# antao97/SegGroup

Measured on AMD Instinct MI355X. Metric: pseudo-label scenes/sec (150k pts, 1.5k segs), higher is better.
Workload: dtype f32 (fp32 accumulate; operands split into 2 x fp16 pieces on v_mfma_f32_32x32x16_f16; kNN / FPS scores in exact fp32 order); 1 GPU; 64 distinct synthetic scenes per GPU per step, 150000 pts / 1500 segs each (BASELINE.json configs[2]; configs[1] = the same scene shape, single scene); mode=ins_infer, scenes_in_flight=112, engine=14 groups x 8 scenes per batched launch, weights=tests/golden/weights_g2.npz, parallelism=scene-parallel x1

## Files before the change

### include/seggroup_hip.h

```cpp
#ifndef SEGGROUP_HIP_H
#define SEGGROUP_HIP_H

#include <stddef.h>
#include <stdint.h>

#ifdef __cplusplus
extern "C" {
#endif

#define SG_OK          0
#define SG_EINVAL     -1
#define SG_EHIP       -2
#define SG_ENOMEM     -3
#define SG_ESTALL     -4
#define SG_EUNSUP     -5
#define SG_EINTERNAL  -6

#define SG_MODE_INS_INFER 0
#define SG_MODE_SEM_INFER 1

#define SG_NUM_LABEL_VECTORS 14
#define SG_RANGE_WORDS 256
#define SG_MAX_POINTS (1 << 20)

const char* sg_last_error(void);
int  sg_version(void);
int  sg_device_count(void);
int  sg_selftest_wave_ops(int* h_mismatches, void* stream);
int  sg_selftest_list_insert(int* h_mismatches, void* stream);

size_t sg_contract_ws_bytes(int S);
int sg_contract_point_edges(const int64_t* d_adj, int E, const int32_t* d_seg_of_point, int N, int S,
                            int32_t* d_out_adj, int out_capacity, int32_t* d_out_count,
                            void* d_ws, size_t ws_bytes, void* stream);

int sg_gather_members(const int32_t* d_seg_points, const int32_t* d_seg_off, int S,
                      const int32_t* d_order, const int32_t* d_dst, const int32_t* d_cl,
                      int32_t* d_members, int32_t* d_pos_of_point, int32_t* d_cluster_of_pos,
                      int32_t* d_slot_of_pos, void* stream);

size_t sg_fps_ws_bytes(int N);
int sg_fps_sample(const float* d_data, int N, int ch_in, const int32_t* d_members, const int32_t* d_cl_off, int C,
                  int P, int ch_out, int transform, float* d_samples, int32_t* d_sel,
                  void* d_ws, size_t ws_bytes, void* stream);

size_t sg_mlp1_ws_bytes(int C);
int sg_mlp1_forward(const float* d_samples, int C, const float* d_w, const float* d_gamma, const float* d_beta,
                    float* d_feat, int feat_stride, void* d_ws, size_t ws_bytes, void* stream);

int sg_edge_distance(const float* d_feat, int feat_stride, int D, const int32_t* d_adj, int E,
                     float* d_dist, void* stream);

int sg_group_max_rows(const float* d_rows, int row_stride, int D, const int32_t* d_goff, const int32_t* d_gidx,
                      int G, float* d_out, int out_stride, void* stream);

int sg_segment_max(const float* d_rows, int N, int D, const int32_t* d_cluster_of_pos,
                   float* d_out, int out_stride, int C, void* stream);

size_t sg_center_ws_bytes(int T, int C);
int sg_center_clusters(const float* d_data, int N, const int32_t* d_members, const int32_t* d_cl_off, int C,
                       const int32_t* d_tile_cl, const int32_t* d_tile_lo, const int32_t* d_tile_hi, int T,
                       const int32_t* d_cl_tile_off, float* d_x9m, float* d_xyzw,
                       void* d_ws, size_t ws_bytes, void* stream);

int sg_cluster_knn(const float* d_xyzw, int N, const int32_t* d_cl_off,
                   const int32_t* d_tile_cl, const int32_t* d_tile_lo, const int32_t* d_tile_hi, int T,
                   int k, int pos0, int32_t* d_knn, void* stream);

int sg_segment_boxes(const float* d_data, const int32_t* d_seg_points, const int32_t* d_seg_off, int S,
                     float* d_box, void* stream);
int sg_cluster_knn_pruned(const float* d_xyzw, int N, const int32_t* d_cl_off,
                          const int32_t* d_tile_cl, const int32_t* d_tile_lo, const int32_t* d_tile_hi, int T,
                          const int32_t* d_cl_seg_off, const int32_t* d_order, const int32_t* d_dst,
                          const int32_t* d_seg_off, const float* d_segbox, const int32_t* d_slot_of_pos,
                          int k, int pos0, int32_t* d_knn, void* stream);

size_t sg_segment_sort_ws_bytes(int N);
int sg_segment_sort_boxes(const float* d_data, int N, const int32_t* d_seg_points, const int32_t* d_seg_off,
                          const int32_t* d_seg_of_point, int S, const int32_t* d_seg_chunk_off, int max_seg, float* d_segbox,
                          int32_t* d_sperm, float* d_chunk_box, double* d_seg_sums, void* d_ws, size_t ws_bytes, void* stream);
int sg_layer_layout(const float* d_data, int N, const int32_t* d_seg_points, const int32_t* d_seg_off, const int32_t* d_sperm, int S,
                    const int32_t* d_order, const int32_t* d_dst, const int32_t* d_cl, const float* d_cl_mean, int32_t* d_members,
                    int32_t* d_pos_of_point, int32_t* d_cluster_of_pos, int32_t* d_slot_of_pos, float* d_x9m, float* d_sxyzw,
                    int32_t* d_smpos, float* d_point_rec, int32_t* d_seed_id, unsigned int* d_range_bits, void* stream);
int sg_knn_operands(const float* d_data, const int32_t* d_seg_points, const int32_t* d_seg_off, const int32_t* d_sperm, int S,
                    const int32_t* d_order, const int32_t* d_dst, float* d_sxyzw, int32_t* d_smpos, void* stream);
int sg_cluster_knn_sorted(const float* d_sxyzw, const int32_t* d_smpos, int N, const int32_t* d_cl_off,
                          const int32_t* d_tile_cl, const int32_t* d_tile_lo, const int32_t* d_tile_hi, int T,
                          const int32_t* d_cl_seg_off, const int32_t* d_order, const int32_t* d_dst,
                          const int32_t* d_seg_off, const int32_t* d_seg_chunk_off, const float* d_segbox,
                          const float* d_chunk_box, const int32_t* d_slot_of_pos, int k, int pos0, int32_t* d_knn, void* stream);
int sg_knn_seed_points(const int32_t* d_knn, const int32_t* d_members, int N, int k, int32_t* d_seed, void* stream);
int sg_cluster_knn_seeded(const float* d_sxyzw, const int32_t* d_smpos, int N, const int32_t* d_cl_off,
                          const int32_t* d_tile_cl, const int32_t* d_tile_lo, const int32_t* d_tile_hi, int T,
                          const int32_t* d_cl_seg_off, const int32_t* d_order, const int32_t* d_dst,
                          const int32_t* d_seg_off, const int32_t* d_seg_chunk_off, const float* d_segbox,
                          const float* d_chunk_box, const int32_t* d_slot_of_pos, const int32_t* d_seed,
                          const int32_t* d_seg_prevcl, const int32_t* d_members, const float* d_point_rec,
                          int k, int pos0, int32_t* d_knn, void* stream);

int sg_knn_chunk_table(const int32_t* d_order, const int32_t* d_dst, const int32_t* d_seg_off, const int32_t* d_seg_chunk_off,
                       const float* d_chunk_box, int S, const int32_t* d_slot_chunk0, float* d_cc, void* stream);
int sg_cluster_knn_2pass(const float* d_sxyzw, const int32_t* d_smpos, int N, const int32_t* d_cl_off,
                         const int32_t* d_tile_cl, const int32_t* d_tile_lo, const int32_t* d_tile_hi,
                         const int32_t* d_tile_chunk0, int T, const int32_t* d_cl_chunk_off, const float* d_cc,
                         int k, int pos0, int32_t* d_knn, void* stream);
int sg_cluster_knn_sorted_w(const float* d_sxyzw, const int32_t* d_smpos, int N, const int32_t* d_cl_off,
                            const int32_t* d_tile_cl, const int32_t* d_tile_lo, const int32_t* d_tile_hi, int T,
                            const int32_t* d_cl_seg_off, const int32_t* d_order, const int32_t* d_dst,
                            const int32_t* d_seg_off, const int32_t* d_seg_chunk_off, const float* d_segbox,
                            const float* d_chunk_box, const int32_t* d_slot_of_pos, int k, int pos0, int waves_per_tile,
                            int32_t* d_knn, void* stream);

size_t sg_edgeconv_ws_bytes(int N);
int sg_edgeconv_forward(const float* d_x9m, const int32_t* d_knn, int N, int k, int layers,
                        const float* d_w1, const float* d_g1, const float* d_b1,
                        const float* d_w2, const float* d_g2, const float* d_b2,
                        float* d_out, void* d_ws, size_t ws_bytes, void* stream);
int sg_edgeconv_forward_r(const float* d_x9m, const int32_t* d_knn, int N, int k, int layers, const float* d_w1, const float* d_g1,
                          const float* d_b1, const float* d_w2, const float* d_g2, const float* d_b2, float* d_out, void* d_ws,
                          size_t ws_bytes, unsigned int* d_range_bits, void* stream);
#define SG_EDGECONV_COMPILER_LOOP 1u
int sg_edgeconv_forward_x(const float* d_x9m, const int32_t* d_knn, int N, int k, int layers, const float* d_w1, const float* d_g1,
                          const float* d_b1, const float* d_w2, const float* d_g2, const float* d_b2, float* d_out, void* d_ws,
                          size_t ws_bytes, unsigned int* d_range_bits, unsigned int flags, void* stream);
int sg_edge_range(const float* d_x9m, int N, unsigned int* d_range_bits, void* stream);

size_t sg_gcn_ws_bytes(int S, int D, int E);
int sg_gcn_forward(const float* d_x, int S, int D, const int32_t* d_adj, int E,
                   const int32_t* d_rowptr, const int32_t* d_col, const int32_t* d_eid,
// ... 527 lines not shown
```

### seggroup_amd/csrc/kernels_knn_sorted.hip

```cpp
#include <cstdlib>


#include "engine_ctx.h"
#include "knn_device.h"
#include "sg_common.h"
#include "wave_ops.h"

namespace {

using namespace sgknn;

#ifdef SG_KNN_PROFILE
constexpr bool kKnnProfile = true;
#else
constexpr bool kKnnProfile = false;
#endif

constexpr int kChunkPts = 32;
constexpr int kQuadS = 4;

__device__ inline unsigned int spread10(unsigned int v);
__device__ inline unsigned int morton30(const float* __restrict__ r, const float* __restrict__ b) {
    const float e[3] = {b[3] - b[0], b[4] - b[1], b[5] - b[2]};
    const float emax = fmaxf(fmaxf(e[0], e[1]), e[2]);
    unsigned int q[3];
#pragma unroll
    for (int k = 0; k < 3; ++k) {
        const float ext = e[k] >= 0.25f * emax ? e[k] : emax;
        const float t = ext > 0.f ? (r[k] - b[k]) / ext : 0.f;
        q[k] = (unsigned int)fminf(fmaxf(t * 1023.f, 0.f), 1023.f);
    }
    return spread10(q[0]) | (spread10(q[1]) << 1) | (spread10(q[2]) << 2);
}

__device__ inline unsigned int spread10(unsigned int v) {
    v &= 0x3ffu;
    v = (v | (v << 16)) & 0x030000ffu;
    v = (v | (v << 8)) & 0x0300f00fu;
    v = (v | (v << 4)) & 0x030c30c3u;
    v = (v | (v << 2)) & 0x09249249u;
    return v;
}

constexpr int kSortCap = sg::kSegMidMax;
__device__ __forceinline__ void segment_sort_boxes_body(const float* __restrict__ data, const int32_t* __restrict__ seg_points,
                                                        const int32_t* __restrict__ seg_off, const int32_t* __restrict__ seg_chunk_off,
                                                        float* __restrict__ segbox, int32_t* __restrict__ sperm,
                                                        float* __restrict__ chunk_box, double* __restrict__ seg_sums, int s) {
    __shared__ unsigned long long key[kSortCap];
    __shared__ float red[4][8];
    __shared__ double dred[4][3];
    __shared__ float bx[8];
    const int tid = threadIdx.x, lane = tid & 63, wave = tid >> 6;
    const int lo = seg_off[s], n = seg_off[s + 1] - lo;
    if (n > kSortCap) return;
    float mn[3] = {INFINITY, INFINITY, INFINITY}, mx[3] = {-INFINITY, -INFINITY, -INFINITY}, xx = 0.f;
    double sm[3] = {0.0, 0.0, 0.0};
    for (int i = tid; i < n; i += 256) {
        const float* r = data + (size_t)seg_points[lo + i] * 6;
#pragma unroll
        for (int k = 0; k < 3; ++k) { mn[k] = fminf(mn[k], r[k]); mx[k] = fmaxf(mx[k], r[k]); sm[k] += (double)r[k]; }
        xx = fmaxf(xx, (r[0] * r[0] + r[1] * r[1]) + r[2] * r[2]);
    }
#pragma unroll
    for (int k = 0; k < 3; ++k) { mn[k] = sgw::wave_min(mn[k]); mx[k] = sgw::wave_max(mx[k]); }
    xx = sgw::wave_max(xx);
    if (seg_sums) {
#pragma unroll
        for (int k = 0; k < 3; ++k) sm[k] = sgw::wave_sum(sm[k]);
        if (lane == 0) { dred[wave][0] = sm[0]; dred[wave][1] = sm[1]; dred[wave][2] = sm[2]; }
    }
    if (lane == 0) { red[wave][0] = mn[0]; red[wave][1] = mn[1]; red[wave][2] = mn[2]; red[wave][3] = mx[0]; red[wave][4] = mx[1]; red[wave][5] = mx[2]; red[wave][6] = xx; }
    __syncthreads();
    if (tid < 7) {
        float v = red[0][tid];
        for (int w = 1; w < 4; ++w) v = tid < 3 ? fminf(v, red[w][tid]) : fmaxf(v, red[w][tid]);
        bx[tid] = v;
        segbox[(size_t)s * 8 + tid] = v;
    }
    if (tid == 7) segbox[(size_t)s * 8 + 7] = 0.f;
    if (seg_sums && tid >= 8 && tid < 11) seg_sums[(size_t)s * 3 + (tid - 8)] = ((dred[0][tid - 8] + dred[1][tid - 8]) + dred[2][tid - 8]) + dred[3][tid - 8];
    __syncthreads();
    int m2 = 64;
    while (m2 < n) m2 <<= 1;
    for (int i = tid; i < m2; i += 256) {
        unsigned long long kk = ~0ull;
        if (i < n) {
            const float* r = data + (size_t)seg_points[lo + i] * 6;
            const unsigned int m = morton30(r, bx);
            kk = ((unsigned long long)m << 32) | (unsigned int)i;
        }
        key[i] = kk;
    }
    __syncthreads();
    for (int k = 2; k <= m2; k <<= 1)
        for (int j = k >> 1; j > 0; j >>= 1) {
            for (int t = tid; t < (m2 >> 1); t += 256) {
                const int i = ((t & ~(j - 1)) << 1) | (t & (j - 1)), p = i | j;
                const unsigned long long a = key[i], b = key[p];
                const bool up = (i & k) == 0;
                if ((a > b) == up) { key[i] = b; key[p] = a; }
            }
            __syncthreads();
        }
    for (int r = tid; r < n; r += 256) sperm[lo + r] = lo + (int)(key[r] & 0xffffffffull);
    const int c0 = seg_chunk_off[s], half = lane >> 5, l = lane & 31;
    for (int j = 2 * wave + half; j * kChunkPts < n; j += 8) {
        const int t = j * kChunkPts + l;
        float cmn[3] = {INFINITY, INFINITY, INFINITY}, cmx[3] = {-INFINITY, -INFINITY, -INFINITY}, cxx = 0.f;
        if (t < n) {
            const float* r = data + (size_t)seg_points[lo + (int)(key[t] & 0xffffffffull)] * 6;
#pragma unroll
            for (int k = 0; k < 3; ++k) { cmn[k] = r[k]; cmx[k] = r[k]; }
            cxx = (r[0] * r[0] + r[1] * r[1]) + r[2] * r[2];
        }
#pragma unroll
        for (int k = 0; k < 3; ++k) { cmn[k] = sgw::half_min(cmn[k], lane); cmx[k] = sgw::half_max(cmx[k], lane); }
        cxx = sgw::half_max(cxx, lane);
        if (l == 0) {
            float* b = chunk_box + (size_t)(c0 + j) * 8;
            b[0] = cmn[0]; b[1] = cmn[1]; b[2] = cmn[2]; b[3] = cmx[0]; b[4] = cmx[1]; b[5] = cmx[2]; b[6] = cxx; b[7] = 0.f;
        }
    }
}
__global__ __launch_bounds__(256) void k_segment_sort_boxes(const float* __restrict__ data, const int32_t* __restrict__ seg_points,
                                                            const int32_t* __restrict__ seg_off, const int32_t* __restrict__ seg_chunk_off,
                                                            float* __restrict__ segbox, int32_t* __restrict__ sperm,
                                                            float* __restrict__ chunk_box, double* __restrict__ seg_sums) {
    segment_sort_boxes_body(data, seg_points, seg_off, seg_chunk_off, segbox, sperm, chunk_box, seg_sums, blockIdx.x);
}
__global__ __launch_bounds__(256) void k_segment_sort_boxes_b(const sg::SlotCtx* __restrict__ cx) {
    const sg::SlotCtx& c = cx[blockIdx.y];
    if ((int)blockIdx.x >= c.S) return;
    segment_sort_boxes_body(c.data, c.seg_points, c.seg_off, c.seg_chunk_off, c.segbox, c.sperm, c.chunk_box, c.seg_sums, blockIdx.x);
}

constexpr int kBigBlock = 1024, kBins = 4096, kWin = 1024;
constexpr int kBigPieces = 16, kPieceBlock = 256;
struct BigScratch {
    float box[kBigPieces][8];
    double sums[kBigPieces][4];
    int hist[kBins];
    int cursor[kBins];
    int first[kBins];
};
static_assert(kBins % kBigPieces == 0 && kBins / kBigPieces == kPieceBlock, "every piece zeroes its own slice of the histogram: one entry per thread");
__host__ __device__ inline size_t bigseg_scratch_slots(int N) { return (size_t)N / (kSortCap + 1) + 1; }
__device__ __forceinline__ BigScratch& bigseg_scratch(unsigned long long* keysA, int N, int lo) {
    return reinterpret_cast<BigScratch*>(keysA + 2 * (size_t)N)[lo / (kSortCap + 1)];
}
__device__ __forceinline__ void piece_range(int n, int piece, int& i0, int& i1) {
    const int L = (n + kBigPieces - 1) / kBigPieces;
    i0 = min(n, piece * L); i1 = min(n, i0 + L);
}

__device__ __forceinline__ void bigseg_box_body(const float* __restrict__ data, const int32_t* __restrict__ seg_points, const int32_t* __restrict__ seg_off,
                                                unsigned long long* __restrict__ keysA, int N, int s, int piece) {
    const int lo = seg_off[s], n = seg_off[s + 1] - lo;
    if (n <= kSortCap) return;
    BigScratch& sc = bigseg_scratch(keysA, N, lo);
    __shared__ float red[kPieceBlock / 64][8];
    __shared__ double dred[kPieceBlock / 64][3];
    const int tid = threadIdx.x, lane = tid & 63, wave = tid >> 6;
    constexpr int kW = kPieceBlock / 64;
    int i0, i1;
    piece_range(n, piece, i0, i1);
    float mn[3] = {INFINITY, INFINITY, INFINITY}, mx[3] = {-INFINITY, -INFINITY, -INFINITY}, xx = 0.f;
    double sm[3] = {0.0, 0.0, 0.0};
#pragma unroll 4
    for (int i = i0 + tid; i < i1; i += kPieceBlock) {
        const float* r = data + (size_t)seg_points[lo + i] * 6;
#pragma unroll
        for (int k = 0; k < 3; ++k) { mn[k] = fminf(mn[k], r[k]); mx[k] = fmaxf(mx[k], r[k]); sm[k] += (double)r[k]; }
        xx = fmaxf(xx, (r[0] * r[0] + r[1] * r[1]) + r[2] * r[2]);
    }
#pragma unroll
    for (int o = 32; o > 0; o >>= 1) {
#pragma unroll
        for (int k = 0; k < 3; ++k) { mn[k] = fminf(mn[k], __shfl_xor(mn[k], o)); mx[k] = fmaxf(mx[k], __shfl_xor(mx[k], o)); sm[k] += __shfl_xor(sm[k], o); }
        xx = fmaxf(xx, __shfl_xor(xx, o));
    }
    if (lane == 0) {
        red[wave][0] = mn[0]; red[wave][1] = mn[1]; red[wave][2] = mn[2]; red[wave][3] = mx[0]; red[wave][4] = mx[1]; red[wave][5] = mx[2]; red[wave][6] = xx;
        dred[wave][0] = sm[0]; dred[wave][1] = sm[1]; dred[wave][2] = sm[2];
    }
    sc.hist[piece * kPieceBlock + tid] = 0;
    sc.cursor[piece * kPieceBlock + tid] = 0;
// ... 929 lines not shown
    for (int j = 0; j < K; ++j) kv[j] = 0ull;
    {
        const unsigned long long floor_key = make_key(floor_score == 0.f ? -0.f : floor_score, 0x7fffffff) & 0xffffffff00000000ull;
        unsigned long long thr = active ? floor_key - 1ull : ~0ull;
        float wk = active ? floor_score : INFINITY;
#pragma unroll
        for (int o = 32; o > 0; o >>= 1) wk = fminf(wk, __shfl_xor(wk, o));
        int cnt = 0;
        auto drain = [&]() {
            int mxc = cnt;
#pragma unroll
            for (int o = 32; o > 0; o >>= 1) mxc = max(mxc, __shfl_xor(mxc, o));
            for (int u = 0; u < mxc; ++u) key_insert<K>(kv, u < cnt ? buf[u][lane] : 0ull);
            cnt = 0;
            if (active && kv[K - 1] > thr) thr = kv[K - 1];
        };
        walk([&]() { return wk; },
             [&](const float* bx) { return !__any(make_key(box_score_bound(me, bx), 0) > thr); },
             [&](float sc, int idx) {
                 const unsigned long long key = make_key(sc, idx);
                 if (key > thr) {
                     buf[cnt][lane] = key;
                     ++cnt;
                 }
             },
             [&]() { return __any(cnt > kBuf2 - kQuadS - 1); }, drain);
    }
    if (active) {
        int32_t* o = knn + (size_t)myrow * K;
#pragma unroll
        for (int j = 0; j < K; ++j) o[j] = clo + key_index(kv[j]);
    }
    if ((dbg & 16) && lane == 0) {
        const unsigned long long t2 = __builtin_readcyclecounter();
        atomicAdd(&g_knn5_stats[0], 1ull);
        atomicAdd(&g_knn5_stats[1], t1 - t0);
        atomicAdd(&g_knn5_stats[3], t2 - t1);
    }
}

}

int sg::knn_variant_for(int T, int override) {
    if (override == 0 || override == 1 || override == 2 || override == 4 || override == 8) return override;
    return T >= 2048 ? 8 : T >= 1024 ? 2 : 4;
}

namespace sg {

bool sort_boxes_fits_lds(int max_seg) { return max_seg <= kSortCap; }

int b_sort_boxes(const SlotCtx* d_ctx, const BatchDims& bd, hipStream_t st, int which) {
    if (bd.nslots == 0 || bd.max_S == 0) return SG_OK;
    if (which & 1) k_segment_sort_boxes_b<<<dim3(bd.max_S, bd.nslots), 256, 0, st>>>(d_ctx);
    if ((which & 2) && bd.max_big > 0) {
        const int wins = sg::cdiv(bd.max_N, kWin);
        k_bigseg_box_b<<<dim3(bd.max_big * kBigPieces, bd.nslots), kPieceBlock, 0, st>>>(d_ctx);
        k_bigseg_keys_b<<<dim3(bd.max_big * kBigPieces, bd.nslots), kPieceBlock, 0, st>>>(d_ctx);
        k_bigseg_scatter_b<<<dim3(bd.max_big * kBigPieces, bd.nslots), kPieceBlock, 0, st>>>(d_ctx);
        k_bigseg_runs_b<<<dim3(wins, bd.nslots), kBigBlock, 0, st>>>(d_ctx);
        k_bigseg_boxes_b<<<dim3(wins, bd.nslots), 512, 0, st>>>(d_ctx);
    }
    SG_LAUNCH_CHECK();
    return SG_OK;
}

int b_layer_layout(const SlotCtx* d_ctx, const BatchDims& bd, hipStream_t st) {
    if (bd.nslots == 0 || bd.max_S == 0) return SG_OK;
    k_layer_layout_b<<<dim3(bd.max_S, bd.nslots), 256, 0, st>>>(d_ctx);
    if (bd.max_lay_big > 0) k_layer_layout_big_b<<<dim3(bd.max_lay_big, bd.nslots), 256, 0, st>>>(d_ctx);
    SG_LAUNCH_CHECK();
    return SG_OK;
}

int b_cluster_knn(const SlotCtx* d_ctx, const BatchDims& bd, int waves_per_tile, bool seeded, hipStream_t st, bool write_seed, bool* wrote_seed) {
    if (wrote_seed) *wrote_seed = false;
    if (bd.nslots == 0 || bd.max_T == 0) return SG_OK;
    if (bd.max_N > sgknn::kListMaxPoints) return sg::fail(SG_EUNSUP, "in-cluster kNN: %d points in a scene, the list keys carry 20 index bits (N <= %d)", bd.max_N, sgknn::kListMaxPoints);
    const dim3 grid(bd.nslots, bd.max_T);
    if (seeded) k_cluster_knn_sorted_b<20, 1, true><<<grid, 64, 0, st>>>(d_ctx, 0);
    else if (waves_per_tile == 1) {
        k_cluster_knn_sorted_b<20, 1, false><<<grid, 64, 0, st>>>(d_ctx, write_seed ? 1 : 0);
        if (wrote_seed) *wrote_seed = write_seed;
    } else if (waves_per_tile == 2) k_cluster_knn_sorted_b<20, 2, false><<<grid, 128, 0, st>>>(d_ctx, 0);
    else k_cluster_knn_sorted_b<20, 4, false><<<grid, 256, 0, st>>>(d_ctx, 0);
    SG_LAUNCH_CHECK();
    return SG_OK;
}

int b_knn_seed_points(const SlotCtx* d_ctx, const BatchDims& bd, hipStream_t st) {
    if (bd.nslots == 0 || bd.max_N == 0) return SG_OK;
    k_knn_seed_points_b<<<dim3(sg::cdiv((long long)bd.max_N * 20, 256), bd.nslots), 256, 0, st>>>(d_ctx);
    SG_LAUNCH_CHECK();
    return SG_OK;
}

}

#ifdef SG_KNN_PROFILE
static int g_knn5_dbg = getenv("SG_KNN_DEBUG") ? atoi(getenv("SG_KNN_DEBUG")) : 0;
#else
static constexpr int g_knn5_dbg = 0;
#endif

extern "C" {

#ifdef SG_KNN_PROFILE
int sg_debug_knn5_stats(unsigned long long* h_out) {
    SG_HIP(hipMemcpyFromSymbol(h_out, HIP_SYMBOL(g_knn5_stats), sizeof(unsigned long long) * 16));
    unsigned long long z[16] = {0};
    SG_HIP(hipMemcpyToSymbol(HIP_SYMBOL(g_knn5_stats), z, sizeof z));
    return SG_OK;
}
#endif

#ifdef SG_KNN_SELFCHECK
int sg_debug_knn_check(unsigned long long* h_out) {
    SG_HIP(hipMemcpyFromSymbol(h_out, HIP_SYMBOL(g_knn_check), sizeof(unsigned long long) * 136));
    unsigned long long z[136] = {0};
    SG_HIP(hipMemcpyToSymbol(HIP_SYMBOL(g_knn_check), z, sizeof z));
    return SG_OK;
}
#endif

size_t sg_segment_sort_ws_bytes(int N) { return sg::align_up((size_t)std::max(N, 1) * 16, 64) + bigseg_scratch_slots(std::max(N, 1)) * sizeof(BigScratch) + 64; }

int sg_layer_layout(const float* d_data, int N, const int32_t* d_seg_points, const int32_t* d_seg_off, const int32_t* d_sperm, int S,
                    const int32_t* d_order, const int32_t* d_dst, const int32_t* d_cl, const float* d_cl_mean, int32_t* d_members,
                    int32_t* d_pos_of_point, int32_t* d_cluster_of_pos, int32_t* d_slot_of_pos, float* d_x9m, float* d_sxyzw,
                    int32_t* d_smpos, float* d_point_rec, int32_t* d_seed_id, unsigned int* d_range_bits, void* stream) {
    SG_REQUIRE(N >= 0 && S >= 0 && d_sperm && d_cl_mean && d_members && d_pos_of_point && d_cluster_of_pos && d_slot_of_pos && d_x9m &&
                   d_sxyzw && d_smpos, "sg_layer_layout: bad arguments");
    if (S == 0) return SG_OK;
    k_layer_layout<<<S, 128, 0, sg::as_stream(stream)>>>(d_data, d_seg_points, d_seg_off, d_sperm, d_order, d_dst, d_cl, d_cl_mean, d_members,
                                                        d_pos_of_point, d_cluster_of_pos, d_slot_of_pos, d_x9m,
                                                        reinterpret_cast<float4*>(d_sxyzw), d_smpos, reinterpret_cast<float4*>(d_point_rec), d_seed_id, d_range_bits);
    SG_LAUNCH_CHECK();
    return SG_OK;
}

int sg_segment_sort_boxes(const float* d_data, int N, const int32_t* d_seg_points, const int32_t* d_seg_off,
                          const int32_t* d_seg_of_point, int S, const int32_t* d_seg_chunk_off, int max_seg, float* d_segbox,
                          int32_t* d_sperm, float* d_chunk_box, double* d_seg_sums, void* d_ws, size_t ws_bytes, void* stream) {
    SG_REQUIRE(N >= 0 && S >= 0 && max_seg >= 0 && d_segbox && d_sperm && d_chunk_box, "sg_segment_sort_boxes: bad arguments");
    if (N == 0 || S == 0) return SG_OK;
    k_segment_sort_boxes<<<S, 256, 0, sg::as_stream(stream)>>>(d_data, d_seg_points, d_seg_off, d_seg_chunk_off, d_segbox, d_sperm, d_chunk_box,
                                                               d_seg_sums);
    if (max_seg > kSortCap) {
        if (!d_ws || ws_bytes < sg_segment_sort_ws_bytes(N)) return sg::fail(SG_ENOMEM, "sg_segment_sort_boxes: workspace too small (%zu < %zu)", ws_bytes, sg_segment_sort_ws_bytes(N));
        unsigned long long* keys = reinterpret_cast<unsigned long long*>(d_ws);
        const int wins = sg::cdiv(N, kWin);
        k_bigseg_box<<<dim3(S, kBigPieces), kPieceBlock, 0, sg::as_stream(stream)>>>(d_data, d_seg_points, d_seg_off, keys, N);
        k_bigseg_keys<<<dim3(S, kBigPieces), kPieceBlock, 0, sg::as_stream(stream)>>>(d_data, d_seg_points, d_seg_off, d_segbox, d_seg_sums, keys, N);
        k_bigseg_scatter<<<dim3(S, kBigPieces), kPieceBlock, 0, sg::as_stream(stream)>>>(d_seg_off, keys, keys + N, N);
        k_bigseg_runs<<<wins, kBigBlock, 0, sg::as_stream(stream)>>>(d_seg_off, S, N, keys, keys + N, d_sperm);
        k_bigseg_boxes<<<wins, 512, 0, sg::as_stream(stream)>>>(d_data, d_seg_points, d_seg_off, S, N, d_seg_chunk_off, d_sperm, d_chunk_box);
    }
    SG_LAUNCH_CHECK();
    return SG_OK;
}

int sg_knn_operands(const float* d_data, const int32_t* d_seg_points, const int32_t* d_seg_off, const int32_t* d_sperm, int S,
                    const int32_t* d_order, const int32_t* d_dst, float* d_sxyzw, int32_t* d_smpos, void* stream) {
    SG_REQUIRE(S >= 0 && d_sxyzw && d_smpos, "sg_knn_operands: bad arguments");
    if (S == 0) return SG_OK;
    k_knn_operands<<<S, 128, 0, sg::as_stream(stream)>>>(d_data, d_seg_points, d_seg_off, d_sperm, d_order, d_dst,
                                                        reinterpret_cast<float4*>(d_sxyzw), d_smpos);
    SG_LAUNCH_CHECK();
    return SG_OK;
}

int sg_knn_seed_points(const int32_t* d_knn, const int32_t* d_members, int N, int k, int32_t* d_seed, void* stream) {
    SG_REQUIRE(N >= 0 && k > 0 && d_knn && d_members && d_seed, "sg_knn_seed_points: bad arguments");
    if (N == 0) return SG_OK;
    k_knn_seed_points<<<sg::cdiv((long long)N * k, 256), 256, 0, sg::as_stream(stream)>>>(d_knn, d_members, N, k, d_seed);
    SG_LAUNCH_CHECK();
    return SG_OK;
}

int sg_cluster_knn_seeded(const float* d_sxyzw, const int32_t* d_smpos, int N, const int32_t* d_cl_off, const int32_t* d_tile_cl,
                          const int32_t* d_tile_lo, const int32_t* d_tile_hi, int T, const int32_t* d_cl_seg_off,
                          const int32_t* d_order, const int32_t* d_dst, const int32_t* d_seg_off, const int32_t* d_seg_chunk_off,
                          const float* d_segbox, const float* d_chunk_box, const int32_t* d_slot_of_pos, const int32_t* d_seed,
                          const int32_t* d_seg_prevcl, const int32_t* d_members, const float* d_point_rec,
                          int k, int pos0, int32_t* d_knn, void* stream) {
    SG_REQUIRE(N >= 0 && T >= 0 && d_knn && d_sxyzw && d_smpos && d_seed && d_seg_prevcl && d_members && d_point_rec,
               "sg_cluster_knn_seeded: bad arguments");
    SG_REQUIRE(N <= sgknn::kListMaxPoints, "sg_cluster_knn_seeded: the list keys carry 20 index bits (N <= 2^20)");
    if (k != 20) return sg::fail(SG_EUNSUP, "sg_cluster_knn_seeded: only k == 20 is built (model.py:788,829), got %d", k);
    if (T == 0) return SG_OK;
    k_cluster_knn_sorted<20, 1, true><<<T, 64, 0, sg::as_stream(stream)>>>(
        reinterpret_cast<const float4*>(d_sxyzw), d_smpos, d_cl_off, d_tile_cl, d_tile_lo, d_tile_hi, d_cl_seg_off, d_order, d_dst,
        d_seg_off, d_seg_chunk_off, d_segbox, d_chunk_box, d_slot_of_pos, pos0, d_knn, g_knn5_dbg, d_seed, d_seg_prevcl, d_members,
        reinterpret_cast<const float4*>(d_point_rec));
    SG_LAUNCH_CHECK();
    return SG_OK;
}

int sg_knn_chunk_table(const int32_t* d_order, const int32_t* d_dst, const int32_t* d_seg_off, const int32_t* d_seg_chunk_off,
                       const float* d_chunk_box, int S, const int32_t* d_slot_chunk0, float* d_cc, void* stream) {
// ... 54 lines not shown
```

### seggroup_amd/csrc/wave_ops.h

```cpp
#pragma once
#include <hip/hip_runtime.h>

namespace sgw {

template <int CTRL, int ROW_MASK = 0xF>
__device__ __forceinline__ int dpp_i(int old, int v) {
    if constexpr (ROW_MASK == 0xF) return __builtin_amdgcn_update_dpp(0, v, CTRL, 0xF, 0xF, true);
    else return __builtin_amdgcn_update_dpp(old, v, CTRL, ROW_MASK, 0xF, false);
}
template <int CTRL, int ROW_MASK = 0xF>
__device__ __forceinline__ float dpp_f(float old, float v) {
    return __int_as_float(dpp_i<CTRL, ROW_MASK>(__float_as_int(old), __float_as_int(v)));
}
template <int CTRL, int ROW_MASK = 0xF>
__device__ __forceinline__ double dpp_d(double old, double v) {
    const long long o = __double_as_longlong(old), x = __double_as_longlong(v);
    const int lo = dpp_i<CTRL, ROW_MASK>((int)(o & 0xffffffffll), (int)(x & 0xffffffffll));
    const int hi = dpp_i<CTRL, ROW_MASK>((int)(o >> 32), (int)(x >> 32));
    return __longlong_as_double(((long long)hi << 32) | (unsigned int)lo);
}

constexpr int kQuadXor1 = 0xB1, kQuadXor2 = 0x4E, kRowRor4 = 0x124, kRowRor8 = 0x128, kRowBcast15 = 0x142, kRowBcast31 = 0x143;

#define SGW_REDUCE(T, DPP, v, OP, IDENT)                                           \
// ... 15 lines not shown
__device__ __forceinline__ float wave_max(float v) {
    SGW_REDUCE(float, dpp_f, v, op_max, v);
    return __int_as_float(__builtin_amdgcn_readlane(__float_as_int(v), 63));
}
__device__ __forceinline__ float wave_min(float v) {
    SGW_REDUCE(float, dpp_f, v, op_min, v);
    return __int_as_float(__builtin_amdgcn_readlane(__float_as_int(v), 63));
}
__device__ __forceinline__ int wave_max(int v) {
    SGW_REDUCE(int, dpp_i, v, op_maxi, v);
    return __builtin_amdgcn_readlane(v, 63);
}
__device__ __forceinline__ float wave_sum(float v) {
    SGW_REDUCE(float, dpp_f, v, op_add, 0.f);
    return __int_as_float(__builtin_amdgcn_readlane(__float_as_int(v), 63));
}
__device__ __forceinline__ double wave_sum(double v) {
    SGW_REDUCE(double, dpp_d, v, op_addd, 0.0);
    const long long x = __double_as_longlong(v);
    const int lo = __builtin_amdgcn_readlane((int)(x & 0xffffffffll), 63), hi = __builtin_amdgcn_readlane((int)(x >> 32), 63);
    return __longlong_as_double(((long long)hi << 32) | (unsigned int)lo);
}

__device__ __forceinline__ int op_mini(int a, int b) { return min(a, b); }
__device__ __forceinline__ int wave_min(int v) {
    SGW_REDUCE(int, dpp_i, v, op_mini, v);
    return __builtin_amdgcn_readlane(v, 63);
}

__device__ __forceinline__ void wave_argmax(float& val, int& idx) {
    const float m = wave_max(val);
    idx = wave_min(val == m ? idx : 0x7fffffff);
    val = m;
}

__device__ __forceinline__ float half_reduce_pick(float v, int lane) {
    const float lo = __int_as_float(__builtin_amdgcn_readlane(__float_as_int(v), 31));
    const float hi = __int_as_float(__builtin_amdgcn_readlane(__float_as_int(v), 63));
    return (lane & 32) ? hi : lo;
}
__device__ __forceinline__ float half_max(float v, int lane) {
    v = fmaxf(v, dpp_f<kQuadXor1>(v, v)); v = fmaxf(v, dpp_f<kQuadXor2>(v, v));
    v = fmaxf(v, dpp_f<kRowRor4>(v, v));  v = fmaxf(v, dpp_f<kRowRor8>(v, v));
    v = fmaxf(v, dpp_f<kRowBcast15, 0xA>(v, v));
    return half_reduce_pick(v, lane);
}
__device__ __forceinline__ float half_min(float v, int lane) {
    v = fminf(v, dpp_f<kQuadXor1>(v, v)); v = fminf(v, dpp_f<kQuadXor2>(v, v));
    v = fminf(v, dpp_f<kRowRor4>(v, v));  v = fminf(v, dpp_f<kRowRor8>(v, v));
    v = fminf(v, dpp_f<kRowBcast15, 0xA>(v, v));
    return half_reduce_pick(v, lane);
}

__device__ __forceinline__ float bcast(float v, int j) { return __int_as_float(__builtin_amdgcn_readlane(__float_as_int(v), j)); }
__device__ __forceinline__ int bcast(int v, int j) { return __builtin_amdgcn_readlane(v, j); }

}
```

### seggroup_amd/hip.py

```python
from __future__ import annotations

import contextlib
import ctypes as C
import os
import struct
import types
from typing import Optional

_HERE = os.path.dirname(os.path.abspath(__file__))
LIB_PATH = os.environ.get("SEGGROUP_HIP_LIB") or os.path.join(_HERE, "libseggroup_hip.so")
HOST_LIB_OVERRIDE = os.environ.get("SEGGROUP_HIP_HOST_LIB")

SG_OK, SG_EINVAL, SG_EHIP, SG_ENOMEM, SG_ESTALL, SG_EUNSUP, SG_EINTERNAL = 0, -1, -2, -3, -4, -5, -6
MODE_INS_INFER, MODE_SEM_INFER = 0, 1
COLOUR_SEMANTIC, COLOUR_INSTANCE, COLOUR_SEGMENT, COLOUR_GROUPING = 0, 1, 2, 3
NUM_LABEL_VECTORS = 14
KNN_BRUTE, KNN_GRID = 0, 1
KNN_INDEX = {"brute": KNN_BRUTE, "grid": KNN_GRID}
MAX_GRID_POINTS = 1 << 24
MAX_POINTS = 1 << 20
MAX_CLOUD_POINTS = 1 << 27
MAX_RADIUS_PAIRS = 1 << 30


# ... 25 lines not shown

class Weights(C.Structure):
    _fields_ = [(n, vp) for n in ("mlp1_w", "mlp1_g", "mlp1_b", "mlp2_w", "mlp2_g", "mlp2_b", "gcn2_w",
                                  "mlp3_w1", "mlp3_g1", "mlp3_b1", "mlp3_w2", "mlp3_g2", "mlp3_b2", "gcn3_w")]


class Scene(C.Structure):
    _fields_ = [("N", C.c_int), ("S", C.c_int), ("E0", C.c_int), ("V", C.c_int),
                ("d_data", vp), ("d_adj", vp), ("d_seg_of_point", vp), ("d_seg_points", vp), ("d_seg_off", vp),
                ("d_unmap", vp), ("d_gt", vp),
                ("h_seg_first", vp), ("h_seg_size", vp), ("h_seg_ins", vp), ("h_seg_sem", vp), ("h_seg_of_vertex", vp)]


class Result(C.Structure):
    _fields_ = [("h_labels", vp), ("iou_sem", C.c_float * 80), ("iou_ins", C.c_float * 80), ("acc", C.c_float * 4),
                ("trace", C.c_int32 * 5), ("stalled", C.c_int32), ("used_fallback", C.c_int32), ("h_tables", vp)]


class Classifier(C.Structure):
    _fields_ = [(n, vp) for n in ("w1", "gamma", "beta", "w2", "b2")]


class Debug(C.Structure):
    _fields_ = [("d_samples1", vp), ("d_feat1", vp), ("d_pointfeat", vp * 2), ("d_knn", vp * 2), ("d_members", vp * 2),
                ("h_gcn", vp * 2), ("h_dist", vp * 3), ("h_adj", vp * 4), ("n_adj", C.c_int32 * 4),
                ("h_feat5", vp), ("h_ins5", vp), ("h_sem5", vp), ("n5", C.c_int32), ("tape", vp), ("d_cat", vp * 2)]


_I, _Z = C.c_int, C.c_size_t
SIGNATURES = {
    "sg_last_error": (C.c_char_p, []),
    "sg_version": (_I, []),
    "sg_device_count": (_I, []),
    "sg_selftest_wave_ops": (_I, [C.POINTER(C.c_int), vp]),
    "sg_selftest_list_insert": (_I, [C.POINTER(C.c_int), vp]),
    "sg_contract_ws_bytes": (_Z, [_I]),
    "sg_contract_point_edges": (_I, [vp, _I, vp, _I, _I, vp, _I, vp, vp, _Z, vp]),
    "sg_gather_members": (_I, [vp, vp, _I, vp, vp, vp, vp, vp, vp, vp, vp]),
    "sg_fps_ws_bytes": (_Z, [_I]),
    "sg_fps_sample": (_I, [vp, _I, _I, vp, vp, _I, _I, _I, _I, vp, vp, vp, _Z, vp]),
    "sg_mlp1_ws_bytes": (_Z, [_I]),
    "sg_mlp1_forward": (_I, [vp, _I, vp, vp, vp, vp, _I, vp, _Z, vp]),
    "sg_edge_distance": (_I, [vp, _I, _I, vp, _I, vp, vp]),
    "sg_group_max_rows": (_I, [vp, _I, _I, vp, vp, _I, vp, _I, vp]),
    "sg_segment_max": (_I, [vp, _I, _I, vp, vp, _I, _I, vp]),
    "sg_center_ws_bytes": (_Z, [_I, _I]),
    "sg_center_clusters": (_I, [vp, _I, vp, vp, _I, vp, vp, vp, _I, vp, vp, vp, vp, _Z, vp]),
    "sg_cluster_knn": (_I, [vp, _I, vp, vp, vp, vp, _I, _I, _I, vp, vp]),
    "sg_segment_boxes": (_I, [vp, vp, vp, _I, vp, vp]),
    "sg_cluster_knn_pruned": (_I, [vp, _I, vp, vp, vp, vp, _I, vp, vp, vp, vp, vp, vp, _I, _I, vp, vp]),
    "sg_segment_sort_ws_bytes": (_Z, [_I]),
    "sg_knn_operands": (_I, [vp, vp, vp, vp, _I, vp, vp, vp, vp, vp]),
    "sg_cluster_knn_sorted": (_I, [vp, vp, _I, vp, vp, vp, vp, _I, vp, vp, vp, vp, vp, vp, vp, vp, _I, _I, vp, vp]),
    "sg_segment_sort_boxes": (_I, [vp, _I, vp, vp, vp, _I, vp, _I, vp, vp, vp, vp, vp, _Z, vp]),
    "sg_layer_layout": (_I, [vp, _I, vp, vp, vp, _I, vp, vp, vp, vp, vp, vp, vp, vp, vp, vp, vp, vp, vp, vp, vp]),
    "sg_cluster_knn_sorted_w": (_I, [vp, vp, _I, vp, vp, vp, vp, _I, vp, vp, vp, vp, vp, vp, vp, vp, _I, _I, _I, vp, vp]),
    "sg_knn_seed_points": (_I, [vp, vp, _I, _I, vp, vp]),
    "sg_cluster_knn_seeded": (_I, [vp, vp, _I, vp, vp, vp, vp, _I, vp, vp, vp, vp, vp, vp, vp, vp, vp, vp, vp, vp, _I, _I, vp, vp]),
    "sg_knn_chunk_table": (_I, [vp, vp, vp, vp, vp, _I, vp, vp, vp]),
    "sg_cluster_knn_2pass": (_I, [vp, vp, _I, vp, vp, vp, vp, vp, _I, vp, vp, _I, _I, vp, vp]),
    "sg_nearest_point_ws_bytes": (_Z, [_I]),
    "sg_nearest_point": (_I, [vp, _I, vp, _I, _I, vp, vp, _Z, vp]),
    "sg_prep_sample_ws_bytes": (_Z, [_I, _I]),
    "sg_prep_sample_points": (_I, [vp, vp, _I, vp, _I, vp, vp, C.POINTER(C.c_int), vp, _Z, vp]),
    "sg_pointcloud_adjacency_ws_bytes": (_Z, [_I, _I]),
    "sg_pointcloud_adjacency": (_I, [vp, _I, _I, _I, vp, C.POINTER(C.c_int), vp, _Z, vp]),
    "sg_mesh_adjacency_ws_bytes": (_Z, [_I]),
    "sg_mesh_adjacency": (_I, [vp, _I, vp, _I, vp, C.POINTER(C.c_int), vp, C.POINTER(C.c_int), vp, _Z, vp]),
    "sg_segment_lists_ws_bytes": (_Z, [_I, _I]),
    "sg_segment_lists": (_I, [vp, _I, vp, _I, vp, vp, vp, C.POINTER(C.c_int), vp, _Z, vp]),
    "sg_write_seg_json": (_I, [C.c_char_p, vp, vp, _I, _I]),
    "sg_overseg_ws_bytes": (_Z, [_I, _I]),
    "sg_overseg_edges": (_I, [vp, _I, vp, _I, vp, vp, vp, vp, C.POINTER(C.c_int), vp, _Z, vp]),
    "sg_overseg_merge": (_I, [vp, vp, _I, _I, C.c_float, _I, vp]),
    "sg_overseg_scan": (_I, [vp, _I, vp, _I, C.c_float, _I, vp, vp, _Z, vp]),
    "sg_overseg_set_timing": (_I, [_I]),
    "sg_overseg_stage_times": (_I, [vp, _I]),
    "sg_overseg_stage_name": (C.c_char_p, [_I]),
    "sg_write_segs_json": (_I, [C.c_char_p, C.c_char_p, vp, _I, C.c_float, _I]),
    "sg_pointcloud_knn_ws_bytes": (_Z, [_I]),
    "sg_pointcloud_knn": (_I, [vp, _I, _I, _I, vp, vp, _Z, vp]),
    "sg_pointcloud_normals": (_I, [vp, _I, vp, _I, vp, vp, vp, _Z, vp]),
    "sg_pcseg_ws_bytes": (_Z, [_I, _I]),
    "sg_pcseg_edges": (_I, [vp, _I, _I, vp, vp, vp, vp, vp, C.POINTER(C.c_int), vp, _Z, vp]),
    "sg_pcseg_scan": (_I, [vp, _I, _I, vp, C.c_float, _I, vp, vp, _Z, vp]),
    "sg_pcseg_set_timing": (_I, [_I]),
    "sg_pcseg_stage_times": (_I, [vp, _I]),
    "sg_pcseg_stage_name": (C.c_char_p, [_I]),
    "sg_cloud_thin_ws_bytes": (_Z, [_I]),
    "sg_cloud_thin": (_I, [vp, _I, _I, C.c_float, vp, vp, C.POINTER(C.c_int), vp, vp, _Z, vp]),
    "sg_cloud_thin_set_timing": (_I, [_I]),
    "sg_cloud_thin_stage_times": (_I, [vp, _I]),
    "sg_cloud_thin_stage_name": (C.c_char_p, [_I]),
    "sg_pointcloud_knn_grid_ws_bytes": (_Z, [_I, _I]),
    "sg_pointcloud_knn_grid": (_I, [vp, _I, _I, _I, C.c_float, vp, vp, _Z, vp]),
    "sg_pointcloud_knn_grid_set_timing": (_I, [_I]),
    "sg_pointcloud_knn_grid_stage_times": (_I, [vp, _I]),
    "sg_pointcloud_knn_grid_stage_name": (C.c_char_p, [_I]),
    "sg_pointcloud_knn_grid_stats": (_I, [vp, _I]),
    "sg_pointcloud_knn_grid_set_tuning": (_I, [_I, _I]),
    "sg_pcseg_ws_bytes_indexed": (_Z, [_I, _I, _I]),
    "sg_pcseg_edges_indexed": (_I, [vp, _I, _I, vp, _I, C.c_float, vp, vp, vp, vp, C.POINTER(C.c_int), vp, _Z, vp]),
    "sg_pcseg_scan_indexed": (_I, [vp, _I, _I, vp, _I, C.c_float, C.c_float, _I, vp, vp, _Z, vp]),
    "sg_nearest_point_grid_ws_bytes": (_Z, [_I, _I]),
    "sg_nearest_point_grid": (_I, [vp, _I, _I, vp, _I, _I, C.c_float, vp, vp, vp, _Z, vp]),
    "sg_nearest_point_grid_set_timing": (_I, [_I]),
# ... 361 lines not shown
```

Baseline: 3562 scenes/s.

## Sort small segments per wave with register bitonic sort instead of per block

Adds a wave-per-segment path for segments of up to 256 points. Each wave loads the points into registers, computes the box and sums with wave reductions, sorts the Morton keys with a register bitonic network built on DPP, swizzle and permlane32, and writes the chunk boxes. Four segments share one block, so small segments no longer occupy a whole 256-thread block with LDS sorting and syncthreads. Larger segments still go to the original block kernel, which now skips any segment the wave kernel handled, at the cost of a second launch when large segments exist.

```diff
diff --git a/include/seggroup_hip.h b/include/seggroup_hip.h
--- a/include/seggroup_hip.h
+++ b/include/seggroup_hip.h
@@ -76,6 +76,8 @@
                           int k, int pos0, int32_t* d_knn, void* stream);
 
 size_t sg_segment_sort_ws_bytes(int N);
+int sg_segment_sort_set_wave_max(int wave_max);
+int sg_segment_sort_get_wave_max(void);
 int sg_segment_sort_boxes(const float* d_data, int N, const int32_t* d_seg_points, const int32_t* d_seg_off,
                           const int32_t* d_seg_of_point, int S, const int32_t* d_seg_chunk_off, int max_seg, float* d_segbox,
                           int32_t* d_sperm, float* d_chunk_box, double* d_seg_sums, void* d_ws, size_t ws_bytes, void* stream);
diff --git a/seggroup_amd/csrc/kernels_knn_sorted.hip b/seggroup_amd/csrc/kernels_knn_sorted.hip
--- a/seggroup_amd/csrc/kernels_knn_sorted.hip
+++ b/seggroup_amd/csrc/kernels_knn_sorted.hip
@@ -1,3 +1,4 @@
+#include <atomic>
 #include <cstdlib>
 
 
@@ -46,7 +47,7 @@
 __device__ __forceinline__ void segment_sort_boxes_body(const float* __restrict__ data, const int32_t* __restrict__ seg_points,
                                                         const int32_t* __restrict__ seg_off, const int32_t* __restrict__ seg_chunk_off,
                                                         float* __restrict__ segbox, int32_t* __restrict__ sperm,
-                                                        float* __restrict__ chunk_box, double* __restrict__ seg_sums, int s) {
+                                                        float* __restrict__ chunk_box, double* __restrict__ seg_sums, int s, int wave_max) {
     __shared__ unsigned long long key[kSortCap];
     __shared__ float red[4][8];
     __shared__ double dred[4][3];
@@ -54,6 +55,7 @@
     const int tid = threadIdx.x, lane = tid & 63, wave = tid >> 6;
     const int lo = seg_off[s], n = seg_off[s + 1] - lo;
     if (n > kSortCap) return;
+    if (wave_max > 0 && n <= wave_max) return;
     float mn[3] = {INFINITY, INFINITY, INFINITY}, mx[3] = {-INFINITY, -INFINITY, -INFINITY}, xx = 0.f;
     double sm[3] = {0.0, 0.0, 0.0};
     for (int i = tid; i < n; i += 256) {
@@ -126,13 +128,193 @@
 __global__ __launch_bounds__(256) void k_segment_sort_boxes(const float* __restrict__ data, const int32_t* __restrict__ seg_points,
                                                             const int32_t* __restrict__ seg_off, const int32_t* __restrict__ seg_chunk_off,
                                                             float* __restrict__ segbox, int32_t* __restrict__ sperm,
-                                                            float* __restrict__ chunk_box, double* __restrict__ seg_sums) {
-    segment_sort_boxes_body(data, seg_points, seg_off, seg_chunk_off, segbox, sperm, chunk_box, seg_sums, blockIdx.x);
-}
-__global__ __launch_bounds__(256) void k_segment_sort_boxes_b(const sg::SlotCtx* __restrict__ cx) {
+                                                            float* __restrict__ chunk_box, double* __restrict__ seg_sums, int wave_max) {
+    segment_sort_boxes_body(data, seg_points, seg_off, seg_chunk_off, segbox, sperm, chunk_box, seg_sums, blockIdx.x, wave_max);
+}
+__global__ __launch_bounds__(256) void k_segment_sort_boxes_b(const sg::SlotCtx* __restrict__ cx, int wave_max) {
     const sg::SlotCtx& c = cx[blockIdx.y];
     if ((int)blockIdx.x >= c.S) return;
-    segment_sort_boxes_body(c.data, c.seg_points, c.seg_off, c.seg_chunk_off, c.segbox, c.sperm, c.chunk_box, c.seg_sums, blockIdx.x);
+    segment_sort_boxes_body(c.data, c.seg_points, c.seg_off, c.seg_chunk_off, c.segbox, c.sperm, c.chunk_box, c.seg_sums, blockIdx.x, wave_max);
+}
+
+constexpr int kWaveCap = 256;
+std::atomic<int> g_wave_max{kWaveCap};
+
+template <int J>
+__device__ __forceinline__ int lane_xor(int v) {
+    static_assert(J == 1 || J == 2 || J == 4 || J == 8 || J == 16, "lane distance");
+    if constexpr (J == 1) return sgw::dpp_i<sgw::kQuadXor1>(v, v);
+    else if constexpr (J == 2) return sgw::dpp_i<sgw::kQuadXor2>(v, v);
+    else if constexpr (J == 8) return sgw::dpp_i<sgw::kRowRor8>(v, v);
+    else return __builtin_amdgcn_ds_swizzle(v, 0x1F | (J << 10));
+}
+constexpr unsigned long long take_min_mask(int K, int J, int u) {
+    unsigned long long m = 0;
+    for (int l = 0; l < 64; ++l) {
+        const int e = l | (u << 6);
+        if (((e & J) == 0) == ((e & K) == 0)) m |= 1ull << l;
+    }
+    return m;
+}
+__device__ __forceinline__ unsigned long long pack64(unsigned int hi, unsigned int lo) { return ((unsigned long long)hi << 32) | lo; }
+
+template <int kU, int K, int J>
+__device__ __forceinline__ void bitonic_pass(unsigned long long (&key)[kU]) {
+    if constexpr (J >= 64) {
+        constexpr int d = J >> 6;
+#pragma unroll
+        for (int u = 0; u < kU; ++u) {
+            if (u & d) continue;
+            const bool up = ((u << 6) & K) == 0;
+            const unsigned long long a = key[u], b = key[u | d];
+            const bool sw = (a > b) == up;
+            key[u] = sw ? b : a;
+            key[u | d] = sw ? a : b;
+        }
+    } else {
+#pragma unroll
+        for (int u = 0; u < kU; ++u) {
+            const bool take_min = __builtin_amdgcn_inverse_ballot_w64(take_min_mask(K, J, u));
+            const unsigned int hi = (unsigned int)(key[u] >> 32), lw = (unsigned int)key[u];
+            unsigned long long a, b;
+            if constexpr (J == 32) {
+                const auto sl = __builtin_amdgcn_permlane32_swap(lw, lw, false, false);
+                const auto sh = __builtin_amdgcn_permlane32_swap(hi, hi, false, false);
+                a = pack64(sh[0], sl[0]);
+                b = pack64(sh[1], sl[1]);
+            } else {
+                a = key[u];
+                b = pack64((unsigned int)lane_xor<J>((int)hi), (unsigned int)lane_xor<J>((int)lw));
+            }
+            key[u] = ((a < b) == take_min) ? a : b;
+        }
+    }
+}
+template <int kU, int K, int J>
+__device__ __forceinline__ void bitonic_merge(unsigned long long (&key)[kU]) {
+    bitonic_pass<kU, K, J>(key);
+    if constexpr (J > 1) bitonic_merge<kU, K, J / 2>(key);
+}
+template <int kU, int K>
+__device__ __forceinline__ void bitonic_sort(unsigned long long (&key)[kU]) {
+    if constexpr (K > 2) bitonic_sort<kU, K / 2>(key);
+    bitonic_merge<kU, K, K / 2>(key);
+}
+
+template <int kU>
+__device__ __forceinline__ void segment_sort_boxes_wave(const float* __restrict__ data, const int32_t* __restrict__ seg_points,
+                                                        const int32_t* __restrict__ seg_chunk_off, float* __restrict__ segbox,
+                                                        int32_t* __restrict__ sperm, float* __restrict__ chunk_box, double* __restrict__ seg_sums,
+                                                        int s, int lo, int n, int lane) {
+    float p[kU][3];
+    const int kPosInf = sgw::ford(INFINITY), kNegInf = sgw::ford(-INFINITY);
+    int omn[3] = {kPosInf, kPosInf, kPosInf}, omx[3] = {kNegInf, kNegInf, kNegInf}, oxx = 0;
+#pragma unroll
+    for (int u = 0; u < kU; ++u) {
+        const int i = lane + 64 * u;
+        p[u][0] = p[u][1] = p[u][2] = 0.f;
+        if (i < n) {
+            const float* r = data + (size_t)seg_points[lo + i] * 6;
+#pragma unroll
+            for (int k = 0; k < 3; ++k) { p[u][k] = r[k]; const int o = sgw::ford(r[k]); omn[k] = min(omn[k], o); omx[k] = max(omx[k], o); }
+            oxx = max(oxx, __float_as_int((r[0] * r[0] + r[1] * r[1]) + r[2] * r[2]));
+        }
+    }
+    float mn[3], mx[3];
+#pragma unroll
+    for (int k = 0; k < 3; ++k) { mn[k] = sgw::ford_back(sgw::wave_min(omn[k])); mx[k] = sgw::ford_back(sgw::wave_max(omx[k])); }
+    const float xx = __int_as_float(sgw::wave_max(oxx));
+    if (seg_sums) {
+        double d[4][3];
+#pragma unroll
+        for (int u = 0; u < 4; ++u)
+#pragma unroll
+            for (int k = 0; k < 3; ++k) {
+                d[u][k] = 0.0;
+                if (u < kU) {
+                    double t = 0.0;
+                    if (lane + 64 * u < n) t += (double)p[u < kU ? u : 0][k];
+                    d[u][k] = sgw::wave_sum(t);
+                }
+            }
+        if (lane == 0) {
+#pragma unroll
+            for (int k = 0; k < 3; ++k) seg_sums[(size_t)s * 3 + k] = ((d[0][k] + d[1][k]) + d[2][k]) + d[3][k];
+        }
+    }
+    if (lane == 0) {
+        float* b = segbox + (size_t)s * 8;
+        b[0] = mn[0]; b[1] = mn[1]; b[2] = mn[2]; b[3] = mx[0]; b[4] = mx[1]; b[5] = mx[2]; b[6] = xx; b[7] = 0.f;
+    }
+    if (n == 0) return;
+    const float bx[6] = {mn[0], mn[1], mn[2], mx[0], mx[1], mx[2]};
+    unsigned long long key[kU];
+#pragma unroll
+    for (int u = 0; u < kU; ++u) {
+        const int i = lane + 64 * u;
+        const unsigned int m = morton30(p[u], bx);
+        key[u] = i < n ? pack64(m, (unsigned int)i) : ~0ull;
+    }
+    bitonic_sort<kU, 64 * kU>(key);
+#pragma unroll
+    for (int u = 0; u < kU; ++u) {
+        const int r = lane + 64 * u;
+        if (r < n) sperm[lo + r] = lo + (int)(unsigned int)key[u];
+    }
+    const int c0 = seg_chunk_off[s], half = lane >> 5, l = lane & 31;
+#pragma unroll
+    for (int u = 0; u < kU; ++u) {
+        if (64 * u >= n) break;
+        const int idx = (int)(unsigned int)key[u], src = (idx & 63) << 2, slot = idx >> 6;
+        float q[3];
+#pragma unroll
+        for (int k = 0; k < 3; ++k) {
+            int g = __builtin_amdgcn_ds_bpermute(src, __float_as_int(p[0][k]));
+#pragma unroll
+            for (int v = 1; v < kU; ++v) {
+                const int t = __builtin_amdgcn_ds_bpermute(src, __float_as_int(p[v][k]));
+                g = slot == v ? t : g;
+            }
+            q[k] = __int_as_float(g);
+        }
+        const int j = 2 * u + half, t = j * kChunkPts + l;
+        int cmn[3] = {kPosInf, kPosInf, kPosInf}, cmx[3] = {kNegInf, kNegInf, kNegInf}, cxx = 0;
+        if (t < n) {
+#pragma unroll
+            for (int k = 0; k < 3; ++k) { cmn[k] = sgw::ford(q[k]); cmx[k] = cmn[k]; }
+            cxx = __float_as_int((q[0] * q[0] + q[1] * q[1]) + q[2] * q[2]);
+        }
+#pragma unroll
+        for (int k = 0; k < 3; ++k) { cmn[k] = sgw::ford(sgw::half_min_tail(cmn[k])); cmx[k] = sgw::ford(sgw::half_max_tail(cmx[k])); }
+        cxx = sgw::half_max_tail(cxx);
+        if (l == 31 && j * kChunkPts < n) {
+            int* b = reinterpret_cast<int*>(chunk_box + (size_t)(c0 + j) * 8);
+            b[0] = cmn[0]; b[1] = cmn[1]; b[2] = cmn[2]; b[3] = cmx[0]; b[4] = cmx[1]; b[5] = cmx[2]; b[6] = cxx; b[7] = 0;
+        }
+    }
+}
+__device__ __forceinline__ void segment_sort_boxes_wave_body(const float* __restrict__ data, const int32_t* __restrict__ seg_points,
+                                                             const int32_t* __restrict__ seg_off, const int32_t* __restrict__ seg_chunk_off,
+                                                             float* __restrict__ segbox, int32_t* __restrict__ sperm,
+                                                             float* __restrict__ chunk_box, double* __restrict__ seg_sums, int S, int wave_max) {
+    const int lane = threadIdx.x & 63;
+    const int s = __builtin_amdgcn_readfirstlane((int)(blockIdx.x * 4 + (threadIdx.x >> 6)));
+    if (s >= S) return;
+    const int lo = seg_off[s], n = seg_off[s + 1] - lo;
+    if (n < 0 || n > wave_max) return;
+    if (n <= 64) segment_sort_boxes_wave<1>(data, seg_points, seg_chunk_off, segbox, sperm, chunk_box, seg_sums, s, lo, n, lane);
+    else if (n <= 128) segment_sort_boxes_wave<2>(data, seg_points, seg_chunk_off, segbox, sperm, chunk_box, seg_sums, s, lo, n, lane);
+    else segment_sort_boxes_wave<4>(data, seg_points, seg_chunk_off, segbox, sperm, chunk_box, seg_sums, s, lo, n, lane);
+}
+__global__ __launch_bounds__(256) void k_segment_sort_boxes_wave(const float* __restrict__ data, const int32_t* __restrict__ seg_points,
+                                                                 const int32_t* __restrict__ seg_off, const int32_t* __restrict__ seg_chunk_off,
+                                                                 float* __restrict__ segbox, int32_t* __restrict__ sperm,
+                                                                 float* __restrict__ chunk_box, double* __restrict__ seg_sums, int S, int wave_max) {
+    segment_sort_boxes_wave_body(data, seg_points, seg_off, seg_chunk_off, segbox, sperm, chunk_box, seg_sums, S, wave_max);
+}
+__global__ __launch_bounds__(256) void k_segment_sort_boxes_wave_b(const sg::SlotCtx* __restrict__ cx, int wave_max) {
+    const sg::SlotCtx& c = cx[blockIdx.y];
+    segment_sort_boxes_wave_body(c.data, c.seg_points, c.seg_off, c.seg_chunk_off, c.segbox, c.sperm, c.chunk_box, c.seg_sums, c.S, wave_max);
 }
 
 constexpr int kBigBlock = 1024, kBins = 4096, kWin = 1024;
@@ -1168,7 +1350,11 @@
 
 int b_sort_boxes(const SlotCtx* d_ctx, const BatchDims& bd, hipStream_t st, int which) {
     if (bd.nslots == 0 || bd.max_S == 0) return SG_OK;
-    if (which & 1) k_segment_sort_boxes_b<<<dim3(bd.max_S, bd.nslots), 256, 0, st>>>(d_ctx);
+    if (which & 1) {
+        const int wave_max = g_wave_max.load();
+        if (wave_max > 0) k_segment_sort_boxes_wave_b<<<dim3(sg::cdiv(bd.max_S, 4), bd.nslots), 256, 0, st>>>(d_ctx, wave_max);
+        if (bd.max_seg > wave_max) k_segment_sort_boxes_b<<<dim3(bd.max_S, bd.nslots), 256, 0, st>>>(d_ctx, wave_max);
+    }
     if ((which & 2) && bd.max_big > 0) {
         const int wins = sg::cdiv(bd.max_N, kWin);
         k_bigseg_box_b<<<dim3(bd.max_big * kBigPieces, bd.nslots), kPieceBlock, 0, st>>>(d_ctx);
@@ -1239,6 +1425,13 @@
 }
 #endif
 
+int sg_segment_sort_set_wave_max(int wave_max) {
+    SG_REQUIRE(wave_max == 0 || wave_max == 64 || wave_max == 128 || wave_max == kWaveCap, "sg_segment_sort_set_wave_max: 0, 64, 128 or %d (%d)", kWaveCap, wave_max);
+    g_wave_max.store(wave_max);
+    return SG_OK;
+}
+int sg_segment_sort_get_wave_max(void) { return g_wave_max.load(); }
+
 size_t sg_segment_sort_ws_bytes(int N) { return sg::align_up((size_t)std::max(N, 1) * 16, 64) + bigseg_scratch_slots(std::max(N, 1)) * sizeof(BigScratch) + 64; }
 
 int sg_layer_layout(const float* d_data, int N, const int32_t* d_seg_points, const int32_t* d_seg_off, const int32_t* d_sperm, int S,
@@ -1260,8 +1453,13 @@
                           int32_t* d_sperm, float* d_chunk_box, double* d_seg_sums, void* d_ws, size_t ws_bytes, void* stream) {
     SG_REQUIRE(N >= 0 && S >= 0 && max_seg >= 0 && d_segbox && d_sperm && d_chunk_box, "sg_segment_sort_boxes: bad arguments");
     if (N == 0 || S == 0) return SG_OK;
-    k_segment_sort_boxes<<<S, 256, 0, sg::as_stream(stream)>>>(d_data, d_seg_points, d_seg_off, d_seg_chunk_off, d_segbox, d_sperm, d_chunk_box,
-                                                               d_seg_sums);
+    const int wave_max = g_wave_max.load();
+    if (wave_max > 0)
+        k_segment_sort_boxes_wave<<<sg::cdiv(S, 4), 256, 0, sg::as_stream(stream)>>>(d_data, d_seg_points, d_seg_off, d_seg_chunk_off, d_segbox, d_sperm,
+                                                                                    d_chunk_box, d_seg_sums, S, wave_max);
+    if (max_seg > wave_max)
+        k_segment_sort_boxes<<<S, 256, 0, sg::as_stream(stream)>>>(d_data, d_seg_points, d_seg_off, d_seg_chunk_off, d_segbox, d_sperm, d_chunk_box,
+                                                                   d_seg_sums, wave_max);
     if (max_seg > kSortCap) {
         if (!d_ws || ws_bytes < sg_segment_sort_ws_bytes(N)) return sg::fail(SG_ENOMEM, "sg_segment_sort_boxes: workspace too small (%zu < %zu)", ws_bytes, sg_segment_sort_ws_bytes(N));
         unsigned long long* keys = reinterpret_cast<unsigned long long*>(d_ws);
diff --git a/seggroup_amd/csrc/wave_ops.h b/seggroup_amd/csrc/wave_ops.h
--- a/seggroup_amd/csrc/wave_ops.h
+++ b/seggroup_amd/csrc/wave_ops.h
@@ -91,6 +91,20 @@
     return half_reduce_pick(v, lane);
 }
 
+__device__ __forceinline__ int ford(int bits) { return bits ^ ((bits >> 31) & 0x7fffffff); }
+__device__ __forceinline__ int ford(float f) { return ford(__float_as_int(f)); }
+__device__ __forceinline__ float ford_back(int o) { return __int_as_float(ford(o)); }
+__device__ __forceinline__ int half_max_tail(int v) {
+    v = max(v, dpp_i<kQuadXor1>(v, v)); v = max(v, dpp_i<kQuadXor2>(v, v));
+    v = max(v, dpp_i<kRowRor4>(v, v));  v = max(v, dpp_i<kRowRor8>(v, v));
+    return max(v, dpp_i<kRowBcast15, 0xA>(v, v));
+}
+__device__ __forceinline__ int half_min_tail(int v) {
+    v = min(v, dpp_i<kQuadXor1>(v, v)); v = min(v, dpp_i<kQuadXor2>(v, v));
+    v = min(v, dpp_i<kRowRor4>(v, v));  v = min(v, dpp_i<kRowRor8>(v, v));
+    return min(v, dpp_i<kRowBcast15, 0xA>(v, v));
+}
+
 __device__ __forceinline__ float bcast(float v, int j) { return __int_as_float(__builtin_amdgcn_readlane(__float_as_int(v), j)); }
 __device__ __forceinline__ int bcast(int v, int j) { return __builtin_amdgcn_readlane(v, j); }
 
diff --git a/seggroup_amd/hip.py b/seggroup_amd/hip.py
--- a/seggroup_amd/hip.py
+++ b/seggroup_amd/hip.py
@@ -101,6 +101,8 @@
     "sg_segment_sort_ws_bytes": (_Z, [_I]),
     "sg_knn_operands": (_I, [vp, vp, vp, vp, _I, vp, vp, vp, vp, vp]),
     "sg_cluster_knn_sorted": (_I, [vp, vp, _I, vp, vp, vp, vp, _I, vp, vp, vp, vp, vp, vp, vp, vp, _I, _I, vp, vp]),
+    "sg_segment_sort_set_wave_max": (_I, [_I]),
+    "sg_segment_sort_get_wave_max": (_I, []),
     "sg_segment_sort_boxes": (_I, [vp, _I, vp, vp, vp, _I, vp, _I, vp, vp, vp, vp, vp, _Z, vp]),
     "sg_layer_layout": (_I, [vp, _I, vp, vp, vp, _I, vp, vp, vp, vp, vp, vp, vp, vp, vp, vp, vp, vp, vp, vp, vp]),
     "sg_cluster_knn_sorted_w": (_I, [vp, vp, _I, vp, vp, vp, vp, _I, vp, vp, vp, vp, vp, vp, vp, vp, _I, _I, _I, vp, vp]),
```

Result: faster. 3612 scenes/s (median of 6 runs) (+1.4%).
